# ikergarcia1996/AI-Generated-GTAV

Measured on NVIDIA B200. Metric: generated frames/sec end-to-end (100-step DiT + VAE decode), higher is better.
Workload: dtype bf16

## Files before the change

### ai-generated-gtav_b200/csrc/attn_mma.cu

```cuda
#include <stdlib.h>

#include "attn_seq.cuh"

namespace gtav {

template <int SEQ, int KB, int WARPS, int ROT_PAIRS>
__global__ void __launch_bounds__(WARPS * 32)
attn_seq_kernel(const bf16* __restrict__ qkv, bf16* __restrict__ out, int heads, const float2* __restrict__ rot) {
    __shared__ __align__(16) bf16 sK[KB * SROW];
    __shared__ __align__(16) bf16 sV[KB * SROW];
    pdl_trigger();
    pdl_wait();
    attn_seq_body<SEQ, KB, WARPS, ROT_PAIRS, false>(qkv, out, heads, rot, sK, sV, blockIdx.x, blockIdx.y, blockIdx.z, threadIdx.x, 0);
}

static constexpr int ROT144_BYTES = 144 * 32 * 8;
static constexpr int ATTN144_SMEM = 2 * 144 * SROW * 2 + ROT144_BYTES;
__global__ void __launch_bounds__(3 * 32)
attn_seq144_kernel(const bf16* __restrict__ qkv, bf16* __restrict__ out, int heads, const float2* __restrict__ rot) {
    extern __shared__ __align__(16) uint8_t smem144[];
    bf16* sK = reinterpret_cast<bf16*>(smem144);
    bf16* sV = sK + 144 * SROW;
    float2* sRot = reinterpret_cast<float2*>(smem144 + 2 * 144 * SROW * 2);
    for (int i = threadIdx.x; i < ROT144_BYTES / 16; i += 3 * 32)
        asm volatile("cp.async.cg.shared.global [%0], [%1], 16;" ::"r"(smem_u32(reinterpret_cast<uint8_t*>(sRot) + i * 16)),
                     "l"(reinterpret_cast<const uint8_t*>(rot) + i * 16) : "memory");
    asm volatile("cp.async.commit_group;" ::: "memory");
    pdl_trigger();
    pdl_wait();
    asm volatile("cp.async.wait_group 0;" ::: "memory");
    __syncthreads();
    attn_seq_body<144, 144, 3, 32, false>(qkv, out, heads, sRot, sK, sV, blockIdx.x, blockIdx.y, blockIdx.z, threadIdx.x, 0);
}

static int attn_use_tc(int seq, int groups) {
    const char* e = getenv("GTAV_ATTN");
    if (e != nullptr && e[0] == 't') return 1;
    if (e != nullptr && e[0] == 'm') return 0;
    return seq == 576 ? groups >= 4 : groups >= 96;
}

int launch_attention_seq(const bf16* qkv, bf16* out, int groups, int seq, int heads, const float2* rot, int rot_pairs,
                         cudaStream_t s) {
    if (groups <= 0) return 0;
    if (((seq == 144 && rot_pairs == 32) || (seq == 576 && rot_pairs == 16)) && attn_use_tc(seq, groups))
        return launch_attention_tc(qkv, out, groups, seq, heads, rot, rot_pairs, s);
    if (seq == 144 && rot_pairs == 32) {
        if (groups * heads * 3 <= 2 * 148) {
            static bool configured = false;
            if (!configured) {
                GTAV_CUDA_OK(cudaFuncSetAttribute(attn_seq144_kernel, cudaFuncAttributeMaxDynamicSharedMemorySize, ATTN144_SMEM));
                configured = true;
            }
            GTAV_CUDA_OK(launch_k(attn_seq144_kernel, dim3(3, heads, groups), dim3(3 * 32), ATTN144_SMEM, s, qkv, out, heads, rot));
        } else {
            GTAV_CUDA_OK(launch_k(attn_seq_kernel<144, 144, 3, 32>, dim3(3, heads, groups), dim3(3 * 32), 0, s, qkv, out, heads, rot));
        }
    } else if (seq == 576 && rot_pairs == 16) {
        GTAV_CUDA_OK(launch_k(attn_seq_kernel<576, 64, 4, 16>, dim3(9, heads, groups), dim3(4 * 32), 0, s, qkv, out, heads, rot));
    } else {
        set_error("attention: unsupported (seq=%d, rot_pairs=%d); built for (144,32) and (576,16)", seq, rot_pairs);
        return -1;
    }
    return 0;
}

}
```

### ai-generated-gtav_b200/csrc/attn_seq.cuh

```cuda
#pragma once
#include "common.cuh"
#include "kernels.h"

namespace gtav {

static constexpr int HD = 64;
static constexpr int SROW = HD + 8;

__device__ __forceinline__ void mma_bf16_16816(float (&d)[4], const uint32_t (&a)[4], uint32_t b0, uint32_t b1) {
    asm volatile(
        "mma.sync.aligned.m16n8k16.row.col.f32.bf16.bf16.f32 {%0,%1,%2,%3}, {%4,%5,%6,%7}, {%8,%9}, {%0,%1,%2,%3};"
        : "+f"(d[0]), "+f"(d[1]), "+f"(d[2]), "+f"(d[3])
        : "r"(a[0]), "r"(a[1]), "r"(a[2]), "r"(a[3]), "r"(b0), "r"(b1));
}
__device__ __forceinline__ void ldmatrix_x4_trans(uint32_t (&r)[4], const void* smem_ptr) {
    asm volatile("ldmatrix.sync.aligned.m8n8.x4.trans.shared.b16 {%0,%1,%2,%3}, [%4];"
                 : "=r"(r[0]), "=r"(r[1]), "=r"(r[2]), "=r"(r[3])
                 : "r"(smem_u32(smem_ptr)));
}
__device__ __forceinline__ uint32_t rotate_pair(uint32_t u, float2 cs) {
    const float2 x = unpack_bf16x2(u);
    return pack_bf16x2(x.x * cs.x - x.y * cs.y, x.y * cs.x + x.x * cs.y);
}


__device__ __forceinline__ void attn_bar(int id, int threads) { asm volatile("bar.sync %0, %1;" ::"r"(id), "r"(threads) : "memory"); }
template <bool COHERENT>
__device__ __forceinline__ uint32_t attn_ld32(const bf16* p) {
    if (COHERENT) return __ldcg(reinterpret_cast<const unsigned int*>(p));
    return *reinterpret_cast<const uint32_t*>(p);
}
template <bool COHERENT>
__device__ __forceinline__ uint4 attn_ld128(const bf16* p) {
    if (COHERENT) return __ldcg(reinterpret_cast<const uint4*>(p));
    return *reinterpret_cast<const uint4*>(p);
}

// ... 165 lines not shown
```

### ai-generated-gtav_b200/csrc/dit_engine.cu

```cuda
#include <stdio.h>
#include <stdlib.h>

#include <new>
#include <vector>

#include "../../include/gtav_b200.h"
#include "kernels.h"

using namespace gtav;

struct gtav_dit_s {
    gtav_dit_config cfg;
    gtav_dit_weights w;
    std::vector<gtav_dit_half> halves;
    int tokens;
    int mod_width;
    int patch_k;
    int out_feat;
};

struct Shape {
    int frames = 0, M = 0;
    GemmOp g_patch, g_final;
    std::vector<GemmOp> g_qkv, g_out, g_fc1, g_fc2;
    std::vector<SkinnyOp> s_qkv, s_out, s_fc1, s_fc2;
    bool sk[4] = {false, false, false, false};
    bool fuse_ln = false, fuse_tattn = false;
};

enum BackboneMode { MODE_FULL = 0, MODE_CONTEXT = 1, MODE_LAST = 2 };

struct gtav_dit_plan_s {
    gtav_dit_t eng;
    int B, T, M, R;
    bf16 *xa, *h, *hn, *qkv, *att, *mlp, *yfin, *temb, *aemb, *h1, *cact, *mod;
    bf16* kv_cache;
    float* sk_ws;
    size_t sk_ws_bytes;
    int* sk_counters;
    bool sk_out_of_step = false;
    GemmOp g_t0, g_t2, g_ada;
    Shape full, ctx, last;
// ... 70 lines not shown
    rc |= gemm_prepare(&sh->g_patch, p->xa, 64, static_cast<const bf16*>(w.patch_w), 64, gp(p->h, D, w.patch_b, M, D, 64), EPI_BIAS);
    const int nh = 2 * h->cfg.depth;
    sh->g_qkv.resize(nh); sh->g_out.resize(nh); sh->g_fc1.resize(nh); sh->g_fc2.resize(nh);
    const bool sk_ok = allow_skinny && skinny_enabled() && p->sk_ws != nullptr;
    sh->sk[0] = sk_ok && skinny_pick_splits(M, 3 * D, D) > 0;
    sh->sk[1] = sk_ok && skinny_pick_splits(M, D, D) > 0;
    sh->sk[2] = sk_ok && skinny_pick_splits(M, 4 * D, D) > 0;
    sh->sk[3] = sk_ok && skinny_pick_splits(M, D, 4 * D) > 0;
    if (sh->sk[0]) sh->s_qkv.resize(nh);
    if (sh->sk[1]) sh->s_out.resize(nh);
    if (sh->sk[2]) sh->s_fc1.resize(nh);
    if (sh->sk[3]) sh->s_fc2.resize(nh);
    int so[4] = {0, 0, 0, 0};
    if (const char* e = getenv("GTAV_SK_SPLITS")) sscanf(e, "%d,%d,%d,%d", &so[0], &so[1], &so[2], &so[3]);
    sh->fuse_ln = sh->sk[1] && sh->sk[3] && fuse_enabled();
    sh->fuse_tattn = sh->sk[0] && fuse_enabled() && (so[0] > 0 ? so[0] : skinny_pick_splits(M, 3 * D, D)) == 4 && p->T - 1 <= 7;
    const size_t cache_layer = static_cast<size_t>(p->B) * (p->T - 1) * S * 2 * D;
    for (int i = 0; i < nh && rc == 0; ++i) {
        const gtav_dit_half& hw = h->halves[i];
        const bf16* modl = p->mod + static_cast<size_t>(i) * 6 * D;
        GemmParams pq = gp(p->qkv, 3 * D, nullptr, M, 3 * D, D);
        GemmParams po = gp(p->h, D, hw.out_b, M, D, D);
        po.res = p->h; po.ldr = D; po.gate = modl + 2 * D; po.gate_ld = W; po.rows_per_frame = S;
        GemmParams p1 = gp(p->mlp, 4 * D, hw.fc1_b, M, 4 * D, D);
        GemmParams p2 = gp(p->h, D, hw.fc2_b, M, D, 4 * D);
        p2.res = p->h; p2.ldr = D; p2.gate = modl + 5 * D; p2.gate_ld = W; p2.rows_per_frame = S;
        const size_t DD = static_cast<size_t>(D) * D * 2;
        const char* pfenv = getenv("GTAV_PREFETCH");
        const bool pf_off = pfenv != nullptr && pfenv[0] == '0', pf_force = pfenv != nullptr && pfenv[0] == '1';
        if (!pf_off) {
            if (pf_force || !sh->sk[0]) { pq.prefetch = hw.out_w; pq.prefetch_bytes = DD; }
            if (pf_force || !sh->sk[1]) { po.prefetch = hw.fc1_w; po.prefetch_bytes = 4 * DD; }
            if (pf_force || !sh->sk[2]) { p1.prefetch = hw.fc2_w; p1.prefetch_bytes = 4 * DD; }
            if ((pf_force || !sh->sk[3]) && i + 1 < nh) { p2.prefetch = h->halves[i + 1].qkv_w; p2.prefetch_bytes = 3 * DD; }
        }
        SkinnyFuseParams f_out{}, f_fc2{}, f_qkv{};
        f_out.mode = f_fc2.mode = SK_FUSE_LN;
        f_out.ln_out = f_fc2.ln_out = p->hn;
        f_out.ln_mod = f_fc2.ln_mod = p->mod;
        f_out.ln_mod_ld = f_fc2.ln_mod_ld = W;
        f_out.ln_shift_off = i * 6 * D + 3 * D; f_out.ln_scale_off = i * 6 * D + 4 * D;
        f_fc2.ln_shift_off = (i + 1) * 6 * D; f_fc2.ln_scale_off = (i + 1) * 6 * D + D;
        f_qkv.mode = SK_FUSE_TATTN;
        f_qkv.kv_cache = p->kv_cache + static_cast<size_t>(i >> 1) * cache_layer;
        f_qkv.rot = reinterpret_cast<const float2*>(w.rot_temporal);
        f_qkv.ctx_frames = p->T - 1;
        f_qkv.positions = S;
        const bool ta = sh->fuse_tattn && (i & 1);
        if (ta) { pq.out = p->att; pq.ldo = D; }
        float* ws4[4];
        for (int k = 0; k < 4; ++k) ws4[k] = reinterpret_cast<float*>(reinterpret_cast<uint8_t*>(p->sk_ws) + k * p->sk_ws_bytes);
        const int tag = tag_enabled() ? (2 | ((i & 1) ^ 1)) : 0;
        if (sh->sk[0]) { rc |= skinny_prepare(&sh->s_qkv[i], p->hn, D, static_cast<const bf16*>(hw.qkv_w), D, pq, EPI_STORE, ws4[0], p->sk_counters, so[0], ta ? &f_qkv : nullptr); sh->s_qkv[i].tag = tag; }
        else rc |= gemm_prepare(&sh->g_qkv[i], p->hn, D, static_cast<const bf16*>(hw.qkv_w), D, pq, EPI_STORE);
        if (sh->sk[1]) { rc |= skinny_prepare(&sh->s_out[i], p->att, D, static_cast<const bf16*>(hw.out_w), D, po, EPI_BIAS_GATE_RES, ws4[1], p->sk_counters, so[1], sh->fuse_ln ? &f_out : nullptr); sh->s_out[i].tag = tag; }
        else rc |= gemm_prepare(&sh->g_out[i], p->att, D, static_cast<const bf16*>(hw.out_w), D, po, EPI_BIAS_GATE_RES);
        if (sh->sk[2]) { rc |= skinny_prepare(&sh->s_fc1[i], p->hn, D, static_cast<const bf16*>(hw.fc1_w), D, p1, EPI_BIAS_GELU_TANH, ws4[2], p->sk_counters, so[2]); sh->s_fc1[i].tag = tag; }
        else rc |= gemm_prepare(&sh->g_fc1[i], p->hn, D, static_cast<const bf16*>(hw.fc1_w), D, p1, EPI_BIAS_GELU_TANH);
        if (sh->sk[3]) { rc |= skinny_prepare(&sh->s_fc2[i], p->mlp, 4 * D, static_cast<const bf16*>(hw.fc2_w), 4 * D, p2, EPI_BIAS_GATE_RES, ws4[3], p->sk_counters, so[3], sh->fuse_ln ? &f_fc2 : nullptr); sh->s_fc2[i].tag = tag; }
        else rc |= gemm_prepare(&sh->g_fc2[i], p->mlp, 4 * D, static_cast<const bf16*>(hw.fc2_w), 4 * D, p2, EPI_BIAS_GATE_RES);
    }
    rc |= gemm_prepare(&sh->g_final, p->hn, D, static_cast<const bf16*>(w.final_w), D, gp(p->yfin, 64, w.final_b, M, h->out_feat, D), EPI_BIAS);
    return rc == 0 ? 0 : (rc < 0 ? rc : -1);
}

int run_backbone(gtav_dit_plan_s* p, const Shape* sh, int mode, const void* x, int x_is_bf16, int first_frame,
                 const int* frame_row, void* out, cudaStream_t stream) {
    const gtav_dit_s* e = p->eng;
// ... 13 lines not shown
    if (const char* tr = getenv("GTAV_ENGINE_TRACE")) trace_base = reinterpret_cast<long long*>(strtoull(tr, nullptr, 0));
    int trace_k = 0;
    auto run_skinny = [&](const SkinnyOp& op0) {
        SkinnyOp o = op0;
        o.p.frame_row = frame_row;
        if (trace_base != nullptr) o.trace = trace_base + static_cast<size_t>(trace_k++) * 160 * 8;
        return skinny_run(&o, stream);
    };
    for (int i = 0; i < 2 * c.depth; ++i) {
        const int off = i * 6 * D;
        if (!hn_ready && (rc = launch_ln_modulate(p->h, p->hn, M, D, p->mod, W, off, off + D, frame_row, S, stream))) return rc;
        if (sh->sk[0]) rc = run_skinny(sh->s_qkv[i]);
        else rc = gemm_run(&sh->g_qkv[i], stream);
        if (rc) return rc;
        if (sh->s_qkv.size() && sh->sk[0] && sh->s_qkv[i].f.mode == SK_FUSE_TATTN) {
        } else if ((i & 1) == 0) {
            rc = launch_attention_seq(p->qkv, p->att, F, S, c.heads, rot_s, 32, stream);
        } else {
            bf16* cache = p->kv_cache + static_cast<size_t>(i >> 1) * cache_layer;
            if (mode == MODE_LAST) rc = launch_attention_temporal_last(p->qkv, p->att, p->B, p->T - 1, S, c.heads, rot_t, cache, stream);
            else rc = launch_attention_temporal(p->qkv, p->att, p->B, sh->frames, S, c.heads, rot_t, mode == MODE_CONTEXT ? cache : nullptr, stream);
        }
        if (rc) return rc;
        if (sh->sk[1]) {
            rc = run_skinny(sh->s_out[i]);
        } else {
            GemmOp o = sh->g_out[i];
            o.p.frame_row = frame_row;
            rc = gemm_run(&o, stream);
        }
// ... 208 lines not shown
                                 gtav_stream_t stream) {
    if (!workspace) { set_error("gemm_skinny_tagged: workspace is required"); return -1; }
    if (parity != 0 && parity != 1) { set_error("gemm_skinny_tagged: parity must be 0 or 1, got %d", parity); return -1; }
    return skinny_standalone(A, lda, W, ldw, out, ldo, M, N, K, epilogue, bias, res, ldr, gate, gate_ld, frame_row, rows_per_frame,
                             splits, workspace, nullptr, 2 | parity, stream);
}

int gtav_gemm_skinny_fused_bf16(const void* A, int lda, const void* W, int ldw, void* out, int ldo, int M, int N, int K,
                                const void* bias, const void* res, int ldr, const void* gate, int gate_ld, const int* frame_row,
                                int splits, void* workspace, int* counters, int mode, void* ln_out, const void* ln_mod,
                                int ln_mod_ld, int ln_shift_off, int ln_scale_off, const void* kv_cache, const float* rot,
                                int ctx_frames, int positions, int parity, gtav_stream_t stream) {
    if (!workspace) { set_error("gemm_skinny_fused: workspace is required"); return -1; }
    if (parity < -1 || parity > 1) { set_error("gemm_skinny_fused: parity must be -1, 0 or 1, got %d", parity); return -1; }
    if (parity == -1 && !counters) { set_error("gemm_skinny_fused: counters are required with parity -1"); return -1; }
    if (mode != SK_FUSE_LN && mode != SK_FUSE_TATTN) { set_error("gemm_skinny_fused: mode must be 1 or 2, got %d", mode); return -1; }
    SkinnyFuseParams f{};
    f.mode = mode;
    f.ln_out = static_cast<bf16*>(ln_out);
    f.ln_mod = static_cast<const bf16*>(ln_mod);
    f.ln_mod_ld = ln_mod_ld; f.ln_shift_off = ln_shift_off; f.ln_scale_off = ln_scale_off;
    f.kv_cache = static_cast<const bf16*>(kv_cache);
    f.rot = reinterpret_cast<const float2*>(rot);
    f.ctx_frames = ctx_frames; f.positions = positions;
    const int epi = mode == SK_FUSE_LN ? EPI_BIAS_GATE_RES : EPI_STORE;
    return skinny_standalone(A, lda, W, ldw, out, ldo, M, N, K, epi, bias, res, ldr, gate, gate_ld, frame_row, 144, splits,
                             workspace, parity == -1 ? counters : nullptr, parity == -1 ? 0 : 2 | parity, stream, &f);
}

int gtav_ln_modulate(const void* x, void* out, int M, int D, const void* mod, int mod_ld, int shift_off, int scale_off,
                     const int* frame_row, int rows_per_frame, gtav_stream_t stream) {
    return launch_ln_modulate(static_cast<const bf16*>(x), static_cast<bf16*>(out), M, D, static_cast<const bf16*>(mod),
                              mod_ld, shift_off, scale_off, frame_row, rows_per_frame, stream);
}
int gtav_ln_affine(const void* x, void* out, int M, int D, const float* w, const float* b, gtav_stream_t stream) {
    return launch_ln_affine(static_cast<const bf16*>(x), static_cast<bf16*>(out), M, D, w, b, stream);
}
int gtav_attention_seq(const void* qkv, void* out, int groups, int seq, int heads, const float* rot, int rot_pairs,
                       gtav_stream_t stream) {
    return launch_attention_seq(static_cast<const bf16*>(qkv), static_cast<bf16*>(out), groups, seq, heads,
                                reinterpret_cast<const float2*>(rot), rot_pairs, stream);
}
int gtav_attention_temporal(const void* qkv, void* out, int B, int T, int positions, int heads, const float* rot,
                            gtav_stream_t stream) {
    return launch_attention_temporal(static_cast<const bf16*>(qkv), static_cast<bf16*>(out), B, T, positions, heads,
                                     reinterpret_cast<const float2*>(rot), nullptr, stream);
}
int gtav_attention_temporal_last(const void* qkv, void* out, int B, int ctx_frames, int positions, int heads,
                                 const float* rot, const void* kv_cache, gtav_stream_t stream) {
    return launch_attention_temporal_last(static_cast<const bf16*>(qkv), static_cast<bf16*>(out), B, ctx_frames, positions,
                                          heads, reinterpret_cast<const float2*>(rot), static_cast<const bf16*>(kv_cache), stream);
}
int gtav_ddim_update(const float* x, const void* v_bf16, float* out, int F, int n, const float* abar_t,
                     const float* abar_next, const int* final_flag, gtav_stream_t stream) {
// ... 5 lines not shown
```

### ai-generated-gtav_b200/csrc/gemm_skinny.cu

```cuda
#include "attn_temporal_core.cuh"
#include "common.cuh"
#include "kernels.h"
#include "ln_row.cuh"

namespace gtav {

static constexpr int SK_THREADS = 256;
static constexpr int SK_NT = 144;
static constexpr int SK_W_CHUNK = 128 * 128;
static constexpr int SK_A_CHUNK = SK_NT * 128;
static constexpr int SK_SMEM_BUDGET = 200 * 1024;
static constexpr int SK_TAIL_BYTES = 128 + 4096 + 2048;
static constexpr int SK_TMAX = 7;

struct SkinnyParams {
    GemmParams g;
    SkinnyFuseParams f;
    int splits, chunks, tiles;
    int gemm_ctas;
    float* ws;
    int* counters;
    int tag;
    long long* trace;
};
// ... 126 lines not shown
        y[3] = r1.y + bf16_round(g1.y * y[3]);
    }
    uint2 o;
    o.x = pack_bf16x2(y[0], y[1]);
    o.y = pack_bf16x2(y[2], y[3]);
    return o;
}
template <int EPI>
__device__ __noinline__ void skinny_store4(const GemmParams& g, int tok, int n, float4 acc, uint2 bias) {
    Epi4Ops e;
    if (EPI == EPI_BIAS_GATE_RES) e = skinny_epi4_load<EPI>(g, tok, n);
    e.bias = bias;
    *reinterpret_cast<uint2*>(g.out + static_cast<size_t>(tok) * g.ldo + n) = skinny_epi4<EPI>(acc, e);
}

template <int EPI, int S>
__device__ __forceinline__ void skinny_reduce(const GemmParams& g, const float* part, int total, int lo, int hi, int wid, int lane,
                                              int n0, uint2 bias, SkTag tg) {
    static_assert(S <= 4, "the unrolled reduce is instantiated for S = 4 only; other split counts use skinny_reduce_any");
    const float* base = part + 4 * lane;
    const uint32_t keep = ~tg.chk;
    constexpr int IT = 5;
#pragma unroll 1
    for (int t0 = lo + wid; t0 < hi; t0 += 8 * IT) {
        uint4 v[IT][S];
        uint32_t pending = 0u, spins = 0u;
#pragma unroll
        for (int it = 0; it < IT; ++it)
#pragma unroll
            for (int s2 = 0; s2 < S; ++s2)
                if (t0 + 8 * it < hi) v[it][s2] = ld_relaxed_u4(base + (static_cast<size_t>(s2) * total + t0 + 8 * it) * 128);
#pragma unroll
        for (int it = 0; it < IT; ++it)
#pragma unroll
            for (int s2 = 0; s2 < S; ++s2)
                if (t0 + 8 * it < hi && !tag_ok(v[it][s2], tg)) pending |= 1u << (S * it + s2);
        while (pending) {
            tag_spin_check(spins);
#pragma unroll
            for (int it = 0; it < IT; ++it)
#pragma unroll
// ... 4 lines not shown
#pragma unroll
                for (int s2 = 0; s2 < S; ++s2)
                    if ((pending >> (S * it + s2) & 1u) && tag_ok(v[it][s2], tg)) pending &= ~(1u << (S * it + s2));
        }
#pragma unroll
        for (int it = 0; it < IT; ++it) {
            const int tok = t0 + 8 * it;
            if (tok < hi) {
                float4 acc = make_float4(__uint_as_float(v[it][0].x & keep), __uint_as_float(v[it][0].y & keep),
                                         __uint_as_float(v[it][0].z & keep), __uint_as_float(v[it][0].w & keep));
#pragma unroll
                for (int s2 = 1; s2 < S; ++s2) {
                    acc.x += __uint_as_float(v[it][s2].x & keep); acc.y += __uint_as_float(v[it][s2].y & keep);
                    acc.z += __uint_as_float(v[it][s2].z & keep); acc.w += __uint_as_float(v[it][s2].w & keep);
                }
                skinny_store4<EPI>(g, tok, n0 + 4 * lane, acc, bias);
            }
        }
    }
}

template <int S>
__device__ __forceinline__ float4 skinny_sum4(const float* p0, size_t stride, SkTag tg) {
    uint4 v[S];
    const uint32_t keep = ~tg.chk;
    uint32_t pending = 0u, spins = 0u;
#pragma unroll
    for (int s2 = 0; s2 < S; ++s2) v[s2] = ld_relaxed_u4(p0 + s2 * stride);
#pragma unroll
    for (int s2 = 0; s2 < S; ++s2)
        if (!tag_ok(v[s2], tg)) pending |= 1u << s2;
// ... 171 lines not shown
    extern __shared__ uint8_t smem_raw[];
    uint8_t* smem = reinterpret_cast<uint8_t*>((reinterpret_cast<uintptr_t>(smem_raw) + 1023) & ~uintptr_t(1023));
    const int chunks = p.chunks, tiles = p.tiles, S = p.splits;
    uint8_t* sW = smem;
    uint8_t* sA = smem + chunks * SK_W_CHUNK;
    uint8_t* tail = sA + tiles * chunks * SK_A_CHUNK;
    uint64_t* bar_w = reinterpret_cast<uint64_t*>(tail);
    uint64_t* bar_a = bar_w + 1;
    uint64_t* bar_acc = bar_w + 6;
    uint32_t* tmem_slot = reinterpret_cast<uint32_t*>(bar_w + 7);
    uint8_t* smod = tail + 128;
    uint8_t* srow = smod + 4096;

    const int warp = threadIdx.x >> 5, lane = threadIdx.x & 31;
    if (threadIdx.x == 128) SK_STAMP(0);
    const bool gemm_cta = FUSE == SK_FUSE_NONE || static_cast<int>(blockIdx.x) < p.gemm_ctas;
    const int rb = blockIdx.x / S, split = blockIdx.x - rb * S;
    const int kc0 = split * chunks;
    const int total = tiles * SK_NT;
    const uint32_t tmem_cols = total <= 256 ? 256u : 512u;
    const bool tagged = p.tag != 0;
    SkTag tg;
    tg.chk = tagged ? 1u : 0u;
    tg.par = tagged ? static_cast<uint32_t>(p.tag & 1) : 0u;

    if (gemm_cta && warp == 0 && lane == 0) {
        tma_prefetch_desc(&tmW);
        mbar_init(bar_w, 1);
        mbar_init(bar_acc, 1);
        fence_barrier_init();
        mbar_arrive_expect_tx(bar_w, chunks * SK_W_CHUNK);
// ... 42 lines not shown
#pragma unroll
                    for (int k = 0; k < 4; ++k)
                        umma_bf16_ss(tmem_base + t * SK_NT, dw + 2 * k, da + 2 * k, idesc, (ch | k) != 0 ? 1u : 0u);
                }
                __syncwarp();
                dw += SK_W_CHUNK >> 4;
                da += SK_A_CHUNK >> 4;
            }
        }
        if (elect_one()) umma_commit(bar_acc);
        __syncwarp();
        pdl_wait();
    } else {
        pdl_wait();
    }
    int* const meet = tagged ? nullptr : p.counters + 4 * (FUSE == SK_FUSE_NONE ? rb : 64);
    const int meet_n = FUSE == SK_FUSE_NONE ? S : static_cast<int>(gridDim.x);
    int sense0 = 0;
    if (threadIdx.x == 128 && meet_n > 1 && !tagged) sense0 = ld_acquire_gpu(meet + 2);
    Epi4Ops epre;
    epre.bias = epre.gate = epre.res = make_uint2(0u, 0u);
    TattnPre tpre;
    if (FUSE == SK_FUSE_LN) {
        if (static_cast<int>(blockIdx.x) < total) epre = skinny_ln_preload(p, blockIdx.x, warp, smod);
    } else if (FUSE == SK_FUSE_TATTN) {
        if (static_cast<int>(blockIdx.x) < total) skinny_tattn_preload(p, blockIdx.x, warp, lane, tpre);
    } else if (EPI != EPI_STORE && S > 1) {
        epre.bias = *reinterpret_cast<const uint2*>(p.g.bias + rb * 128 + 4 * lane);
    }

    if (FUSE == SK_FUSE_NONE && S == 1 && warp >= 4) {
        const GemmParams& g = p.g;
        const int q = warp & 3;
        const int n = rb * 128 + q * 32 + lane;
        float bias_n = 0.f;
        if (EPI != EPI_STORE) bias_n = __bfloat162float(g.bias[n]);
        mbar_wait(bar_acc, 0);
        tcgen05_fence_after();
        const uint32_t tlane = tmem_base + (static_cast<uint32_t>(q * 32) << 16);
#pragma unroll 1
        for (int c = 0; c < total; c += 16) {
            uint32_t v[16];
            tmem_ld_32x16(tlane + c, v);
            tmem_ld_wait();
#pragma unroll
            for (int i = 0; i < 16; ++i) skinny_store<EPI>(g, c + i, n, __uint_as_float(v[i]), bias_n);
// ... 42 lines not shown
            if (threadIdx.x == 128) SK_STAMP(5);
            const long long t0 = clock64();
            tcgen05_fence_before();
            if (warp == 2) {
                asm volatile("bar.sync 1, 256;" ::: "memory");
                tcgen05_fence_after();
                tmem_dealloc(tmem_base, tmem_cols);
            } else {
                asm volatile("bar.arrive 1, 256;" ::: "memory");
            }
            if (GTAV_SK_TAG_DELAY > 0) {
                while (clock64() - t0 < GTAV_SK_TAG_DELAY) {}
            }
            if (threadIdx.x == 128) SK_STAMP(6);
        }
    } else if (FUSE != SK_FUSE_NONE && !tagged && threadIdx.x == 128) {
        skinny_rendezvous(meet, meet_n, sense0);
    } else if (FUSE != SK_FUSE_NONE && tagged) {
        if (threadIdx.x == 0 && static_cast<int>(blockIdx.x) < total) {
            const float* probe = p.ws + (static_cast<size_t>(p.gemm_ctas - 1) * total + blockIdx.x) * 128 + 127;
            uint32_t spins = 0u;
            while (!tag_ok(ld_relaxed_u1(probe), tg)) tag_spin_check(spins);
        }
        __syncthreads();
    }
    if (S > 1 && FUSE == SK_FUSE_NONE) {
        if (!tagged) {
            __syncthreads();
            if (threadIdx.x == 128) SK_STAMP(6);
        }
        const GemmParams& g = p.g;
        const int lo = split * total / S, hi = (split + 1) * total / S;
        const float* part = p.ws + static_cast<size_t>(rb) * S * total * 128;
        if (S == 4) skinny_reduce<EPI, 4>(g, part, total, lo, hi, warp, lane, rb * 128, epre.bias, tg);
        else skinny_reduce_any<EPI>(g, part, S, total, lo, hi, warp, lane, rb * 128, epre.bias, tg);
        if (threadIdx.x == 128) SK_STAMP(7);
    }
    if (FUSE != SK_FUSE_NONE) {
        if (!tagged) {
            __syncthreads();
            if (threadIdx.x == 128) SK_STAMP(6);
        }
        if (FUSE == SK_FUSE_LN) {
            skinny_reduce_ln(p, S, total, warp, lane, smod, srow, epre, tg);
        } else {
            skinny_reduce_tattn<4>(p, total, warp, lane, tpre, tg);
        }
        if (threadIdx.x == 128) SK_STAMP(7);
    }
    if (S == 1 && gemm_cta) {
        tcgen05_fence_before();
        __syncthreads();
        if (warp == 2) tmem_dealloc(tmem_base, tmem_cols);
// ... 52 lines not shown
    op->splits = S;
    op->chunks = kchunks / S;
    op->tiles = tiles;
    op->ws = ws;
    op->counters = counters;
    op->trace = nullptr;
    op->tag = 0;
    op->f = SkinnyFuseParams{};
    op->grid = rbs * S;
    if (fuse != nullptr && fuse->mode != SK_FUSE_NONE) {
        const bool ln_ok = fuse->mode == SK_FUSE_LN && epi == EPI_BIAS_GATE_RES && p.N == 1024 && (S == 4 || S == 8 || S == 16) && fuse->ln_out != nullptr &&
                           fuse->ln_mod != nullptr && fuse->ln_mod_ld % 8 == 0 && fuse->ln_shift_off % 8 == 0 && fuse->ln_scale_off % 8 == 0;
        const bool ta_ok = fuse->mode == SK_FUSE_TATTN && epi == EPI_STORE && p.N == 3072 && S == 4 && fuse->rot != nullptr &&
                           fuse->ctx_frames >= 0 && fuse->ctx_frames <= 7 && (fuse->ctx_frames == 0 || fuse->kv_cache != nullptr) &&
                           fuse->positions > 0 && p.M % fuse->positions == 0;
        if (!ln_ok && !ta_ok) {
            set_error("skinny gemm: fused reduce mode %d does not fit M=%d N=%d K=%d epi=%d splits=%d", fuse->mode, p.M, p.N, p.K, epi, S);
            return -1;
        }
        op->f = *fuse;
        int sms = 148, dev = 0, n = 0;
        if (cudaGetDevice(&dev) == cudaSuccess && cudaDeviceGetAttribute(&n, cudaDevAttrMultiProcessorCount, dev) == cudaSuccess && n > 0) sms = n;
        const int want = p.M < sms ? p.M : sms;
        if (want > op->grid) op->grid = want;
    }
    int rc = make_tmap_3d(&op->tmW, W, p.N, p.K, ldw, 128, op->chunks);
    if (rc) return rc;
    return make_tmap_3d(&op->tmA, A, p.M, p.K, lda, SK_NT, op->chunks);
}

template <int EPI, int FUSE>
static int skinny_launch(const SkinnyOp* op, cudaStream_t stream) {
    static bool configured = false;
    auto kern = gemm_skinny_kernel<EPI, FUSE>;
    if (!configured) {
// ... 2 lines not shown
    }
    SkinnyParams sp;
    sp.g = op->p; sp.f = op->f; sp.splits = op->splits; sp.chunks = op->chunks; sp.tiles = op->tiles; sp.ws = op->ws;
    sp.counters = op->counters; sp.gemm_ctas = (op->p.N / 128) * op->splits;
    sp.trace = op->trace;
    sp.tag = op->tag;
    size_t smem = static_cast<size_t>(op->chunks) * (SK_W_CHUNK + op->tiles * SK_A_CHUNK) + SK_TAIL_BYTES + 1024;
    if (smem < 120 * 1024) smem = 120 * 1024;
    GTAV_CUDA_OK(launch_k(kern, dim3(op->grid), dim3(SK_THREADS), smem, stream, op->tmW, op->tmA, sp));
    return 0;
}

int skinny_run(const SkinnyOp* op, cudaStream_t stream) {
    if (op->f.mode == SK_FUSE_LN) return skinny_launch<EPI_BIAS_GATE_RES, SK_FUSE_LN>(op, stream);
    if (op->f.mode == SK_FUSE_TATTN) return skinny_launch<EPI_STORE, SK_FUSE_TATTN>(op, stream);
    switch (op->epi) {
        case EPI_STORE: return skinny_launch<EPI_STORE, SK_FUSE_NONE>(op, stream);
        case EPI_BIAS: return skinny_launch<EPI_BIAS, SK_FUSE_NONE>(op, stream);
        case EPI_BIAS_GELU_TANH: return skinny_launch<EPI_BIAS_GELU_TANH, SK_FUSE_NONE>(op, stream);
        case EPI_BIAS_GATE_RES: return skinny_launch<EPI_BIAS_GATE_RES, SK_FUSE_NONE>(op, stream);
    }
    set_error("skinny gemm: unknown epilogue %d", op->epi);
    return -1;
}

}
```

### ai-generated-gtav_b200/csrc/kernels.h

```cpp
#pragma once
#include <cuda.h>
#include <cuda_bf16.h>
#include <cuda_runtime.h>
#include <stdint.h>

namespace gtav {

typedef __nv_bfloat16 bf16;

void set_error(const char* fmt, ...);
const char* get_error();
#define GTAV_CUDA_OK(expr)                                                                     \
    do {                                                                                       \
        cudaError_t e__ = (expr);                                                              \
        if (e__ != cudaSuccess) {                                                              \
            gtav::set_error("%s failed: %s (%s:%d)", #expr, cudaGetErrorString(e__), __FILE__, __LINE__); \
            return -2;                                                                         \
        }                                                                                      \
    } while (0)

bool pdl_enabled();
template <typename... KArgs, typename... Args>
inline cudaError_t launch_k(void (*kern)(KArgs...), dim3 grid, dim3 block, size_t smem, cudaStream_t stream, Args&&... args) {
    cudaLaunchConfig_t cfg{};
// ... 43 lines not shown
    int kc;
    int epi;
};

int gemm_prepare(GemmOp* op, const bf16* A, int lda, const bf16* W, int ldw, const GemmParams& p, int epi,
                 int bn_override = 0);
int gemm_run(const GemmOp* op, cudaStream_t stream);
bool gemm2_eligible(int M, int N, int K);
int gemm2_run(const GemmOp* op, cudaStream_t stream);
bool gemm_splitk_eligible(int M, int N, int K, int sms);
int gemm_splitk_run(const GemmOp* op, cudaStream_t stream);

int make_tmap_3d(CUtensorMap* out, const bf16* ptr, uint64_t rows, uint64_t cols, uint64_t ld, uint32_t box_rows,
                 uint32_t box_chunks);

enum SkinnyFuse : int { SK_FUSE_NONE = 0, SK_FUSE_LN = 1, SK_FUSE_TATTN = 2 };
struct SkinnyFuseParams {
    int mode;
    bf16* ln_out;
    const bf16* ln_mod;
    int ln_mod_ld, ln_shift_off, ln_scale_off;
    const bf16* kv_cache;
    const float2* rot;
    int ctx_frames, positions;
};
struct SkinnyOp {
    CUtensorMap tmW, tmA;
    GemmParams p;
    SkinnyFuseParams f;
    int grid;
    int epi, splits, chunks, tiles;
// ... 3 lines not shown
    long long* trace;
};
bool skinny_supported(int M, int N, int K, int epi);
int skinny_pick_splits(int M, int N, int K);
size_t skinny_workspace_bytes(int M);
int skinny_prepare(SkinnyOp* op, const bf16* A, int lda, const bf16* W, int ldw, const GemmParams& p, int epi, float* ws,
                   int* counters, int splits_override = 0, const SkinnyFuseParams* fuse = nullptr);
int skinny_run(const SkinnyOp* op, cudaStream_t stream);

int launch_ln_modulate(const bf16* x, bf16* out, int M, int D, const bf16* mod, int mod_ld, int shift_off,
                       int scale_off, const int* frame_row, int rows_per_frame, cudaStream_t s);
int launch_ln_affine(const bf16* x, bf16* out, int M, int D, const float* w, const float* b, cudaStream_t s);

int launch_attention_seq(const bf16* qkv, bf16* out, int groups, int seq, int heads, const float2* rot, int rot_pairs,
                         cudaStream_t s);
int launch_attention_tc(const bf16* qkv, bf16* out, int groups, int seq, int heads, const float2* rot, int rot_pairs,
                        cudaStream_t s);
int launch_attention_temporal(const bf16* qkv, bf16* out, int B, int T, int positions, int heads, const float2* rot,
                              bf16* kv_cache, cudaStream_t s);
int launch_attention_temporal_last(const bf16* qkv, bf16* out, int B, int ctx_frames, int positions, int heads,
                                   const float2* rot, const bf16* kv_cache, cudaStream_t s);

int launch_cond_prep(const int64_t* t, const float* actions, int act_dim, int R, const float* freqs, const bf16* Wa,
                     const bf16* ba, bf16* temb, bf16* aemb, int D, cudaStream_t s);
int launch_patchify(const void* x, int x_is_bf16, bf16* out, int ldo, int F, int C, int H, int W, int p,
                    int frames_per_group, long group_stride, cudaStream_t s);
int launch_dit_unpatchify(const bf16* y, bf16* out, int F, int C, int gh, int gw, int p, cudaStream_t s);
int launch_vae_unpatchify(const bf16* y, void* out, int to_u8, int F, int sh, int sw, int p, cudaStream_t s);
int launch_cast_pad(const float* z, bf16* out, int rows, int C, int ldo, float scale, cudaStream_t s);
int launch_take_mean(const bf16* moments, int ldm, float* out, int rows, int C, float scale, int round_bf16,
// ... 10 lines not shown
```

Baseline: 10.03.

## Fuse spatial RoPE into skinny QKV reduce and add key-split seq-144 attention

Adds a new seq-144 spatial attention kernel that splits the keys across three warps, each handling 48 keys, and merges the partial softmax results through shared memory, with a finer grid (9 query blocks per head). Adds a skinny-GEMM fusion mode that applies the spatial rotary rotation to the Q/K columns during the split-K reduce, so the attention kernel can skip the rotation. The engine turns both on whenever the QKV skinny GEMM uses 4 splits. This is meant to cut attention latency and rotation work per step, at the cost of an extra cross-warp merge and rounding the rotated values to bf16 at a different point.

```diff
diff --git a/ai-generated-gtav_b200/csrc/attn_mma.cu b/ai-generated-gtav_b200/csrc/attn_mma.cu
--- a/ai-generated-gtav_b200/csrc/attn_mma.cu
+++ b/ai-generated-gtav_b200/csrc/attn_mma.cu
@@ -33,6 +33,176 @@
     attn_seq_body<144, 144, 3, 32, false>(qkv, out, heads, sRot, sK, sV, blockIdx.x, blockIdx.y, blockIdx.z, threadIdx.x, 0);
 }
 
+static constexpr int A144_KEYS = 48;
+template <bool ROTATE>
+__global__ void __launch_bounds__(3 * 32)
+attn_seq144_split_kernel(const bf16* __restrict__ qkv, bf16* __restrict__ out, int heads, const float2* __restrict__ rot) {
+    __shared__ __align__(16) bf16 sK[144 * SROW];
+    __shared__ __align__(16) bf16 sV[144 * SROW];
+    __shared__ __align__(16) bf16 sQ[3][16 * SROW];
+    const int warp = threadIdx.x >> 5, lane = threadIdx.x & 31;
+    const int g = lane >> 2, tig = lane & 3;
+    const int q0 = blockIdx.x * 16, head = blockIdx.y, k0 = warp * A144_KEYS;
+    const int ld = 3 * heads * HD;
+    const bf16* qbase = qkv + static_cast<size_t>(blockIdx.z) * 144 * ld + head * HD;
+    const bf16* kbase = qbase + heads * HD;
+    const bf16* vbase = kbase + heads * HD;
+    bf16* myQ = sQ[warp];
+    bf16* myK = sK + k0 * SROW;
+    bf16* myV = sV + k0 * SROW;
+    constexpr int QC = 16 * 8 / 32, KC = A144_KEYS * 8 / 32;
+    float4 cs[QC + KC][2];
+    if (ROTATE) {
+#pragma unroll
+        for (int i = 0; i < QC + KC; ++i) {
+            const int idx = lane + 32 * (i < QC ? i : i - QC);
+            const int r = (i < QC ? q0 : k0) + (idx >> 3), c8 = (idx & 7) * 8;
+            const float4* t = reinterpret_cast<const float4*>(rot + r * 32 + (c8 >> 1));
+            cs[i][0] = __ldg(t);
+            cs[i][1] = __ldg(t + 1);
+        }
+    }
+    pdl_trigger();
+    pdl_wait();
+#pragma unroll
+    for (int i = 0; i < QC + KC; ++i) {
+        const int idx = lane + 32 * (i < QC ? i : i - QC);
+        const int r = idx >> 3, c8 = (idx & 7) * 8;
+        const bf16* src = i < QC ? qbase + static_cast<size_t>(q0 + r) * ld + c8 : kbase + static_cast<size_t>(k0 + r) * ld + c8;
+        bf16* dst = (i < QC ? myQ : myK) + r * SROW + c8;
+        asm volatile("cp.async.cg.shared.global [%0], [%1], 16;" ::"r"(smem_u32(dst)), "l"(src) : "memory");
+    }
+    asm volatile("cp.async.commit_group;" ::: "memory");
+#pragma unroll
+    for (int i = 0; i < KC; ++i) {
+        const int idx = lane + 32 * i;
+        const int r = idx >> 3, c8 = (idx & 7) * 8;
+        asm volatile("cp.async.cg.shared.global [%0], [%1], 16;" ::"r"(smem_u32(myV + r * SROW + c8)),
+                     "l"(vbase + static_cast<size_t>(k0 + r) * ld + c8) : "memory");
+    }
+    asm volatile("cp.async.commit_group;" ::: "memory");
+    asm volatile("cp.async.wait_group 1;" ::: "memory");
+    if (ROTATE) {
+#pragma unroll
+        for (int i = 0; i < QC + KC; ++i) {
+            const int idx = lane + 32 * (i < QC ? i : i - QC);
+            const int r = idx >> 3, c8 = (idx & 7) * 8;
+            uint4* p = reinterpret_cast<uint4*>((i < QC ? myQ : myK) + r * SROW + c8);
+            uint4 x = *p;
+            x.x = rotate_pair(x.x, make_float2(cs[i][0].x, cs[i][0].y));
+            x.y = rotate_pair(x.y, make_float2(cs[i][0].z, cs[i][0].w));
+            x.z = rotate_pair(x.z, make_float2(cs[i][1].x, cs[i][1].y));
+            x.w = rotate_pair(x.w, make_float2(cs[i][1].z, cs[i][1].w));
+            *p = x;
+        }
+    }
+    __syncwarp();
+
+    uint32_t qf[4][4];
+#pragma unroll
+    for (int ks = 0; ks < 4; ++ks)
+#pragma unroll
+        for (int h = 0; h < 4; ++h)
+            qf[ks][h] = *reinterpret_cast<const uint32_t*>(myQ + (g + (h & 1) * 8) * SROW + ks * 16 + 2 * tig + (h >> 1) * 8);
+    float sc[A144_KEYS / 8][4];
+#pragma unroll
+    for (int nt = 0; nt < A144_KEYS / 8; ++nt) {
+#pragma unroll
+        for (int j = 0; j < 4; ++j) sc[nt][j] = 0.f;
+#pragma unroll
+        for (int ks = 0; ks < 4; ++ks) {
+            const bf16* kp = myK + (nt * 8 + g) * SROW + ks * 16 + 2 * tig;
+            mma_bf16_16816(sc[nt], qf[ks], *reinterpret_cast<const uint32_t*>(kp), *reinterpret_cast<const uint32_t*>(kp + 8));
+        }
+    }
+    const float sl2 = 0.125f * 1.4426950408889634f;
+    float m[2] = {-INFINITY, -INFINITY}, l[2] = {0.f, 0.f};
+#pragma unroll
+    for (int nt = 0; nt < A144_KEYS / 8; ++nt) {
+        m[0] = fmaxf(m[0], fmaxf(sc[nt][0], sc[nt][1]));
+        m[1] = fmaxf(m[1], fmaxf(sc[nt][2], sc[nt][3]));
+    }
+#pragma unroll
+    for (int h = 0; h < 2; ++h) {
+        m[h] = fmaxf(m[h], __shfl_xor_sync(0xffffffffu, m[h], 1));
+        m[h] = fmaxf(m[h], __shfl_xor_sync(0xffffffffu, m[h], 2));
+    }
+    const float mo0 = m[0] * sl2, mo1 = m[1] * sl2;
+#pragma unroll
+    for (int nt = 0; nt < A144_KEYS / 8; ++nt) {
+        sc[nt][0] = exp2f(sc[nt][0] * sl2 - mo0);
+        sc[nt][1] = exp2f(sc[nt][1] * sl2 - mo0);
+        sc[nt][2] = exp2f(sc[nt][2] * sl2 - mo1);
+        sc[nt][3] = exp2f(sc[nt][3] * sl2 - mo1);
+        l[0] += sc[nt][0] + sc[nt][1];
+        l[1] += sc[nt][2] + sc[nt][3];
+    }
+#pragma unroll
+    for (int h = 0; h < 2; ++h) {
+        l[h] += __shfl_xor_sync(0xffffffffu, l[h], 1);
+        l[h] += __shfl_xor_sync(0xffffffffu, l[h], 2);
+    }
+    float o[8][4];
+#pragma unroll
+    for (int i = 0; i < 8; ++i)
+#pragma unroll
+        for (int j = 0; j < 4; ++j) o[i][j] = 0.f;
+    asm volatile("cp.async.wait_group 0;" ::: "memory");
+    __syncwarp();
+#pragma unroll
+    for (int j = 0; j < A144_KEYS / 16; ++j) {
+        uint32_t pf[4];
+        pf[0] = pack_bf16x2(sc[2 * j][0], sc[2 * j][1]);
+        pf[1] = pack_bf16x2(sc[2 * j][2], sc[2 * j][3]);
+        pf[2] = pack_bf16x2(sc[2 * j + 1][0], sc[2 * j + 1][1]);
+        pf[3] = pack_bf16x2(sc[2 * j + 1][2], sc[2 * j + 1][3]);
+#pragma unroll
+        for (int dn = 0; dn < 8; dn += 2) {
+            const int mat = lane >> 3, r = lane & 7;
+            uint32_t vf[4];
+            ldmatrix_x4_trans(vf, myV + (j * 16 + (mat & 1) * 8 + r) * SROW + (dn + (mat >> 1)) * 8);
+            mma_bf16_16816(o[dn], pf, vf[0], vf[1]);
+            mma_bf16_16816(o[dn + 1], pf, vf[2], vf[3]);
+        }
+    }
+    if (warp > 0) {
+        float4* x = reinterpret_cast<float4*>(myK);
+#pragma unroll
+        for (int i = 0; i < 8; ++i) x[i * 32 + lane] = make_float4(o[i][0], o[i][1], o[i][2], o[i][3]);
+        x[8 * 32 + lane] = make_float4(m[0], m[1], l[0], l[1]);
+    }
+    __syncthreads();
+    if (warp > 0) return;
+    const float4* x1 = reinterpret_cast<const float4*>(sK + A144_KEYS * SROW);
+    const float4* x2 = reinterpret_cast<const float4*>(sK + 2 * A144_KEYS * SROW);
+    const float4 ml1 = x1[8 * 32 + lane], ml2 = x2[8 * 32 + lane];
+    float a[3][2], inv[2];
+    {
+        const float mm[3][2] = {{m[0], m[1]}, {ml1.x, ml1.y}, {ml2.x, ml2.y}};
+        const float ll[3][2] = {{l[0], l[1]}, {ml1.z, ml1.w}, {ml2.z, ml2.w}};
+#pragma unroll
+        for (int h = 0; h < 2; ++h) {
+            const float mx = fmaxf(fmaxf(mm[0][h], mm[1][h]), mm[2][h]);
+#pragma unroll
+            for (int w = 0; w < 3; ++w) a[w][h] = exp2f((mm[w][h] - mx) * sl2);
+            inv[h] = 1.0f / (ll[0][h] * a[0][h] + ll[1][h] * a[1][h] + ll[2][h] * a[2][h]);
+        }
+    }
+    const int ldo = heads * HD;
+    bf16* obase = out + (static_cast<size_t>(blockIdx.z) * 144 + q0) * ldo + head * HD;
+#pragma unroll
+    for (int dn = 0; dn < 8; ++dn) {
+        const float4 y1 = x1[dn * 32 + lane], y2 = x2[dn * 32 + lane];
+        const float r0 = o[dn][0] * a[0][0] + y1.x * a[1][0] + y2.x * a[2][0];
+        const float r1 = o[dn][1] * a[0][0] + y1.y * a[1][0] + y2.y * a[2][0];
+        const float r2 = o[dn][2] * a[0][1] + y1.z * a[1][1] + y2.z * a[2][1];
+        const float r3 = o[dn][3] * a[0][1] + y1.w * a[1][1] + y2.w * a[2][1];
+        const int c = dn * 8 + 2 * tig;
+        *reinterpret_cast<uint32_t*>(obase + static_cast<size_t>(g) * ldo + c) = pack_bf16x2(r0 * inv[0], r1 * inv[0]);
+        *reinterpret_cast<uint32_t*>(obase + static_cast<size_t>(g + 8) * ldo + c) = pack_bf16x2(r2 * inv[1], r3 * inv[1]);
+    }
+}
+
 static int attn_use_tc(int seq, int groups) {
     const char* e = getenv("GTAV_ATTN");
     if (e != nullptr && e[0] == 't') return 1;
@@ -43,6 +213,8 @@
 int launch_attention_seq(const bf16* qkv, bf16* out, int groups, int seq, int heads, const float2* rot, int rot_pairs,
                          cudaStream_t s) {
     if (groups <= 0) return 0;
+    const char* e = getenv("GTAV_ATTN");
+    if (seq == 144 && rot_pairs == 32 && e != nullptr && e[0] == 's') return launch_attention_seq144_split(qkv, out, groups, heads, rot, s);
     if (((seq == 144 && rot_pairs == 32) || (seq == 576 && rot_pairs == 16)) && attn_use_tc(seq, groups))
         return launch_attention_tc(qkv, out, groups, seq, heads, rot, rot_pairs, s);
     if (seq == 144 && rot_pairs == 32) {
@@ -65,4 +237,11 @@
     return 0;
 }
 
-}
+int launch_attention_seq144_split(const bf16* qkv, bf16* out, int groups, int heads, const float2* rot, cudaStream_t s) {
+    if (groups <= 0) return 0;
+    if (rot != nullptr) GTAV_CUDA_OK(launch_k(attn_seq144_split_kernel<true>, dim3(9, heads, groups), dim3(3 * 32), 0, s, qkv, out, heads, rot));
+    else GTAV_CUDA_OK(launch_k(attn_seq144_split_kernel<false>, dim3(9, heads, groups), dim3(3 * 32), 0, s, qkv, out, heads, rot));
+    return 0;
+}
+
+}
diff --git a/ai-generated-gtav_b200/csrc/attn_seq.cuh b/ai-generated-gtav_b200/csrc/attn_seq.cuh
--- a/ai-generated-gtav_b200/csrc/attn_seq.cuh
+++ b/ai-generated-gtav_b200/csrc/attn_seq.cuh
@@ -20,7 +20,7 @@
 }
 __device__ __forceinline__ uint32_t rotate_pair(uint32_t u, float2 cs) {
     const float2 x = unpack_bf16x2(u);
-    return pack_bf16x2(x.x * cs.x - x.y * cs.y, x.y * cs.x + x.x * cs.y);
+    return pack_bf16x2(__fmaf_rn(x.x, cs.x, -__fmul_rn(x.y, cs.y)), __fmaf_rn(x.y, cs.x, __fmul_rn(x.x, cs.y)));
 }
 
 
diff --git a/ai-generated-gtav_b200/csrc/dit_engine.cu b/ai-generated-gtav_b200/csrc/dit_engine.cu
--- a/ai-generated-gtav_b200/csrc/dit_engine.cu
+++ b/ai-generated-gtav_b200/csrc/dit_engine.cu
@@ -25,7 +25,8 @@
     std::vector<GemmOp> g_qkv, g_out, g_fc1, g_fc2;
     std::vector<SkinnyOp> s_qkv, s_out, s_fc1, s_fc2;
     bool sk[4] = {false, false, false, false};
-    bool fuse_ln = false, fuse_tattn = false;
+    bool fuse_ln = false, fuse_tattn = false, fuse_rot = false;
+    bool attn_split = false;
 };
 
 enum BackboneMode { MODE_FULL = 0, MODE_CONTEXT = 1, MODE_LAST = 2 };
@@ -126,7 +127,9 @@
     int so[4] = {0, 0, 0, 0};
     if (const char* e = getenv("GTAV_SK_SPLITS")) sscanf(e, "%d,%d,%d,%d", &so[0], &so[1], &so[2], &so[3]);
     sh->fuse_ln = sh->sk[1] && sh->sk[3] && fuse_enabled();
-    sh->fuse_tattn = sh->sk[0] && fuse_enabled() && (so[0] > 0 ? so[0] : skinny_pick_splits(M, 3 * D, D)) == 4 && p->T - 1 <= 7;
+    sh->attn_split = sh->sk[0] && (so[0] > 0 ? so[0] : skinny_pick_splits(M, 3 * D, D)) == 4;
+    sh->fuse_rot = sh->attn_split && fuse_enabled();
+    sh->fuse_tattn = sh->fuse_rot && p->T - 1 <= 7;
     const size_t cache_layer = static_cast<size_t>(p->B) * (p->T - 1) * S * 2 * D;
     for (int i = 0; i < nh && rc == 0; ++i) {
         const gtav_dit_half& hw = h->halves[i];
@@ -146,7 +149,7 @@
             if (pf_force || !sh->sk[2]) { p1.prefetch = hw.fc2_w; p1.prefetch_bytes = 4 * DD; }
             if ((pf_force || !sh->sk[3]) && i + 1 < nh) { p2.prefetch = h->halves[i + 1].qkv_w; p2.prefetch_bytes = 3 * DD; }
         }
-        SkinnyFuseParams f_out{}, f_fc2{}, f_qkv{};
+        SkinnyFuseParams f_out{}, f_fc2{}, f_qkv{}, f_rot{};
         f_out.mode = f_fc2.mode = SK_FUSE_LN;
         f_out.ln_out = f_fc2.ln_out = p->hn;
         f_out.ln_mod = f_fc2.ln_mod = p->mod;
@@ -158,12 +161,15 @@
         f_qkv.rot = reinterpret_cast<const float2*>(w.rot_temporal);
         f_qkv.ctx_frames = p->T - 1;
         f_qkv.positions = S;
+        f_rot.mode = SK_FUSE_ROT;
+        f_rot.rot = reinterpret_cast<const float2*>(w.rot_spatial);
         const bool ta = sh->fuse_tattn && (i & 1);
+        const SkinnyFuseParams* fq = ta ? &f_qkv : (sh->fuse_rot && !(i & 1) ? &f_rot : nullptr);
         if (ta) { pq.out = p->att; pq.ldo = D; }
         float* ws4[4];
         for (int k = 0; k < 4; ++k) ws4[k] = reinterpret_cast<float*>(reinterpret_cast<uint8_t*>(p->sk_ws) + k * p->sk_ws_bytes);
         const int tag = tag_enabled() ? (2 | ((i & 1) ^ 1)) : 0;
-        if (sh->sk[0]) { rc |= skinny_prepare(&sh->s_qkv[i], p->hn, D, static_cast<const bf16*>(hw.qkv_w), D, pq, EPI_STORE, ws4[0], p->sk_counters, so[0], ta ? &f_qkv : nullptr); sh->s_qkv[i].tag = tag; }
+        if (sh->sk[0]) { rc |= skinny_prepare(&sh->s_qkv[i], p->hn, D, static_cast<const bf16*>(hw.qkv_w), D, pq, EPI_STORE, ws4[0], p->sk_counters, so[0], fq); sh->s_qkv[i].tag = tag; }
         else rc |= gemm_prepare(&sh->g_qkv[i], p->hn, D, static_cast<const bf16*>(hw.qkv_w), D, pq, EPI_STORE);
         if (sh->sk[1]) { rc |= skinny_prepare(&sh->s_out[i], p->att, D, static_cast<const bf16*>(hw.out_w), D, po, EPI_BIAS_GATE_RES, ws4[1], p->sk_counters, so[1], sh->fuse_ln ? &f_out : nullptr); sh->s_out[i].tag = tag; }
         else rc |= gemm_prepare(&sh->g_out[i], p->att, D, static_cast<const bf16*>(hw.out_w), D, po, EPI_BIAS_GATE_RES);
@@ -207,6 +213,8 @@
         else rc = gemm_run(&sh->g_qkv[i], stream);
         if (rc) return rc;
         if (sh->s_qkv.size() && sh->sk[0] && sh->s_qkv[i].f.mode == SK_FUSE_TATTN) {
+        } else if ((i & 1) == 0 && sh->attn_split) {
+            rc = launch_attention_seq144_split(p->qkv, p->att, F, c.heads, sh->s_qkv[i].f.mode == SK_FUSE_ROT ? nullptr : rot_s, stream);
         } else if ((i & 1) == 0) {
             rc = launch_attention_seq(p->qkv, p->att, F, S, c.heads, rot_s, 32, stream);
         } else {
@@ -445,7 +453,10 @@
     if (!workspace) { set_error("gemm_skinny_fused: workspace is required"); return -1; }
     if (parity < -1 || parity > 1) { set_error("gemm_skinny_fused: parity must be -1, 0 or 1, got %d", parity); return -1; }
     if (parity == -1 && !counters) { set_error("gemm_skinny_fused: counters are required with parity -1"); return -1; }
-    if (mode != SK_FUSE_LN && mode != SK_FUSE_TATTN) { set_error("gemm_skinny_fused: mode must be 1 or 2, got %d", mode); return -1; }
+    if (mode != SK_FUSE_LN && mode != SK_FUSE_TATTN && mode != SK_FUSE_ROT) {
+        set_error("gemm_skinny_fused: mode must be 1, 2 or 3, got %d", mode);
+        return -1;
+    }
     SkinnyFuseParams f{};
     f.mode = mode;
     f.ln_out = static_cast<bf16*>(ln_out);
@@ -469,6 +480,10 @@
 }
 int gtav_attention_seq(const void* qkv, void* out, int groups, int seq, int heads, const float* rot, int rot_pairs,
                        gtav_stream_t stream) {
+    if (rot == nullptr) {
+        if (seq != 144) { set_error("attention_seq: q / k arrive rotated (rot NULL) for seq 144 only, got %d", seq); return -1; }
+        return launch_attention_seq144_split(static_cast<const bf16*>(qkv), static_cast<bf16*>(out), groups, heads, nullptr, stream);
+    }
     return launch_attention_seq(static_cast<const bf16*>(qkv), static_cast<bf16*>(out), groups, seq, heads,
                                 reinterpret_cast<const float2*>(rot), rot_pairs, stream);
 }
diff --git a/ai-generated-gtav_b200/csrc/gemm_skinny.cu b/ai-generated-gtav_b200/csrc/gemm_skinny.cu
--- a/ai-generated-gtav_b200/csrc/gemm_skinny.cu
+++ b/ai-generated-gtav_b200/csrc/gemm_skinny.cu
@@ -1,3 +1,4 @@
+#include "attn_seq.cuh"
 #include "attn_temporal_core.cuh"
 #include "common.cuh"
 #include "kernels.h"
@@ -164,9 +165,19 @@
     *reinterpret_cast<uint2*>(g.out + static_cast<size_t>(tok) * g.ldo + n) = skinny_epi4<EPI>(acc, e);
 }
 
-template <int EPI, int S>
+__device__ __forceinline__ void skinny_store4_rot(const GemmParams& g, int tok, int n, float4 acc, bool rotq, float4 cs) {
+    Epi4Ops e;
+    uint2 o = skinny_epi4<EPI_STORE>(acc, e);
+    if (rotq) {
+        o.x = rotate_pair(o.x, make_float2(cs.x, cs.y));
+        o.y = rotate_pair(o.y, make_float2(cs.z, cs.w));
+    }
+    *reinterpret_cast<uint2*>(g.out + static_cast<size_t>(tok) * g.ldo + n) = o;
+}
+
+template <int EPI, int S, bool ROT = false>
 __device__ __forceinline__ void skinny_reduce(const GemmParams& g, const float* part, int total, int lo, int hi, int wid, int lane,
-                                              int n0, uint2 bias, SkTag tg) {
+                                              int n0, uint2 bias, SkTag tg, const float2* rot = nullptr) {
     static_assert(S <= 4, "the unrolled reduce is instantiated for S = 4 only; other split counts use skinny_reduce_any");
     const float* base = part + 4 * lane;
     const uint32_t keep = ~tg.chk;
@@ -175,6 +186,13 @@
     for (int t0 = lo + wid; t0 < hi; t0 += 8 * IT) {
         uint4 v[IT][S];
         uint32_t pending = 0u, spins = 0u;
+        const bool rotq = ROT && n0 < 2048;
+        float4 cs[IT];
+        if (rotq) {
+#pragma unroll
+            for (int it = 0; it < IT; ++it)
+                if (t0 + 8 * it < hi) cs[it] = __ldg(reinterpret_cast<const float4*>(rot + ((t0 + 8 * it) % SK_NT) * 32 + (((n0 + 4 * lane) & 63) >> 1)));
+        }
 #pragma unroll
         for (int it = 0; it < IT; ++it)
 #pragma unroll
@@ -209,7 +227,8 @@
                     acc.x += __uint_as_float(v[it][s2].x & keep); acc.y += __uint_as_float(v[it][s2].y & keep);
                     acc.z += __uint_as_float(v[it][s2].z & keep); acc.w += __uint_as_float(v[it][s2].w & keep);
                 }
-                skinny_store4<EPI>(g, tok, n0 + 4 * lane, acc, bias);
+                if (ROT) skinny_store4_rot(g, tok, n0 + 4 * lane, acc, rotq, cs[it]);
+                else skinny_store4<EPI>(g, tok, n0 + 4 * lane, acc, bias);
             }
         }
     }
@@ -411,7 +430,8 @@
 
     const int warp = threadIdx.x >> 5, lane = threadIdx.x & 31;
     if (threadIdx.x == 128) SK_STAMP(0);
-    const bool gemm_cta = FUSE == SK_FUSE_NONE || static_cast<int>(blockIdx.x) < p.gemm_ctas;
+    constexpr bool ROWS = FUSE == SK_FUSE_LN || FUSE == SK_FUSE_TATTN;
+    const bool gemm_cta = !ROWS || static_cast<int>(blockIdx.x) < p.gemm_ctas;
     const int rb = blockIdx.x / S, split = blockIdx.x - rb * S;
     const int kc0 = split * chunks;
     const int total = tiles * SK_NT;
@@ -484,8 +504,8 @@
     } else {
         pdl_wait();
     }
-    int* const meet = tagged ? nullptr : p.counters + 4 * (FUSE == SK_FUSE_NONE ? rb : 64);
-    const int meet_n = FUSE == SK_FUSE_NONE ? S : static_cast<int>(gridDim.x);
+    int* const meet = tagged ? nullptr : p.counters + 4 * (!ROWS ? rb : 64);
+    const int meet_n = !ROWS ? S : static_cast<int>(gridDim.x);
     int sense0 = 0;
     if (threadIdx.x == 128 && meet_n > 1 && !tagged) sense0 = ld_acquire_gpu(meet + 2);
     Epi4Ops epre;
@@ -499,7 +519,7 @@
         epre.bias = *reinterpret_cast<const uint2*>(p.g.bias + rb * 128 + 4 * lane);
     }
 
-    if (FUSE == SK_FUSE_NONE && S == 1 && warp >= 4) {
+    if (!ROWS && S == 1 && warp >= 4) {
         const GemmParams& g = p.g;
         const int q = warp & 3;
         const int n = rb * 128 + q * 32 + lane;
@@ -572,9 +592,9 @@
             }
             if (threadIdx.x == 128) SK_STAMP(6);
         }
-    } else if (FUSE != SK_FUSE_NONE && !tagged && threadIdx.x == 128) {
+    } else if (ROWS && !tagged && threadIdx.x == 128) {
         skinny_rendezvous(meet, meet_n, sense0);
-    } else if (FUSE != SK_FUSE_NONE && tagged) {
+    } else if (ROWS && tagged) {
         if (threadIdx.x == 0 && static_cast<int>(blockIdx.x) < total) {
             const float* probe = p.ws + (static_cast<size_t>(p.gemm_ctas - 1) * total + blockIdx.x) * 128 + 127;
             uint32_t spins = 0u;
@@ -582,7 +602,7 @@
         }
         __syncthreads();
     }
-    if (S > 1 && FUSE == SK_FUSE_NONE) {
+    if (S > 1 && !ROWS) {
         if (!tagged) {
             __syncthreads();
             if (threadIdx.x == 128) SK_STAMP(6);
@@ -590,11 +610,12 @@
         const GemmParams& g = p.g;
         const int lo = split * total / S, hi = (split + 1) * total / S;
         const float* part = p.ws + static_cast<size_t>(rb) * S * total * 128;
-        if (S == 4) skinny_reduce<EPI, 4>(g, part, total, lo, hi, warp, lane, rb * 128, epre.bias, tg);
+        if (FUSE == SK_FUSE_ROT) skinny_reduce<EPI, 4, true>(g, part, total, lo, hi, warp, lane, rb * 128, epre.bias, tg, p.f.rot);
+        else if (S == 4) skinny_reduce<EPI, 4>(g, part, total, lo, hi, warp, lane, rb * 128, epre.bias, tg);
         else skinny_reduce_any<EPI>(g, part, S, total, lo, hi, warp, lane, rb * 128, epre.bias, tg);
         if (threadIdx.x == 128) SK_STAMP(7);
     }
-    if (FUSE != SK_FUSE_NONE) {
+    if (ROWS) {
         if (!tagged) {
             __syncthreads();
             if (threadIdx.x == 128) SK_STAMP(6);
@@ -677,11 +698,14 @@
         const bool ta_ok = fuse->mode == SK_FUSE_TATTN && epi == EPI_STORE && p.N == 3072 && S == 4 && fuse->rot != nullptr &&
                            fuse->ctx_frames >= 0 && fuse->ctx_frames <= 7 && (fuse->ctx_frames == 0 || fuse->kv_cache != nullptr) &&
                            fuse->positions > 0 && p.M % fuse->positions == 0;
-        if (!ln_ok && !ta_ok) {
+        const bool rot_ok = fuse->mode == SK_FUSE_ROT && epi == EPI_STORE && p.N == 3072 && S == 4 && fuse->rot != nullptr;
+        if (!ln_ok && !ta_ok && !rot_ok) {
             set_error("skinny gemm: fused reduce mode %d does not fit M=%d N=%d K=%d epi=%d splits=%d", fuse->mode, p.M, p.N, p.K, epi, S);
             return -1;
         }
         op->f = *fuse;
+    }
+    if (fuse != nullptr && (fuse->mode == SK_FUSE_LN || fuse->mode == SK_FUSE_TATTN)) {
         int sms = 148, dev = 0, n = 0;
         if (cudaGetDevice(&dev) == cudaSuccess && cudaDeviceGetAttribute(&n, cudaDevAttrMultiProcessorCount, dev) == cudaSuccess && n > 0) sms = n;
         const int want = p.M < sms ? p.M : sms;
@@ -714,6 +738,7 @@
 int skinny_run(const SkinnyOp* op, cudaStream_t stream) {
     if (op->f.mode == SK_FUSE_LN) return skinny_launch<EPI_BIAS_GATE_RES, SK_FUSE_LN>(op, stream);
     if (op->f.mode == SK_FUSE_TATTN) return skinny_launch<EPI_STORE, SK_FUSE_TATTN>(op, stream);
+    if (op->f.mode == SK_FUSE_ROT) return skinny_launch<EPI_STORE, SK_FUSE_ROT>(op, stream);
     switch (op->epi) {
         case EPI_STORE: return skinny_launch<EPI_STORE, SK_FUSE_NONE>(op, stream);
         case EPI_BIAS: return skinny_launch<EPI_BIAS, SK_FUSE_NONE>(op, stream);
diff --git a/ai-generated-gtav_b200/csrc/kernels.h b/ai-generated-gtav_b200/csrc/kernels.h
--- a/ai-generated-gtav_b200/csrc/kernels.h
+++ b/ai-generated-gtav_b200/csrc/kernels.h
@@ -81,7 +81,7 @@
 int make_tmap_3d(CUtensorMap* out, const bf16* ptr, uint64_t rows, uint64_t cols, uint64_t ld, uint32_t box_rows,
                  uint32_t box_chunks);
 
-enum SkinnyFuse : int { SK_FUSE_NONE = 0, SK_FUSE_LN = 1, SK_FUSE_TATTN = 2 };
+enum SkinnyFuse : int { SK_FUSE_NONE = 0, SK_FUSE_LN = 1, SK_FUSE_TATTN = 2, SK_FUSE_ROT = 3 };
 struct SkinnyFuseParams {
     int mode;
     bf16* ln_out;
@@ -115,6 +115,7 @@
 
 int launch_attention_seq(const bf16* qkv, bf16* out, int groups, int seq, int heads, const float2* rot, int rot_pairs,
                          cudaStream_t s);
+int launch_attention_seq144_split(const bf16* qkv, bf16* out, int groups, int heads, const float2* rot, cudaStream_t s);
 int launch_attention_tc(const bf16* qkv, bf16* out, int groups, int seq, int heads, const float2* rot, int rot_pairs,
                         cudaStream_t s);
 int launch_attention_temporal(const bf16* qkv, bf16* out, int B, int T, int positions, int heads, const float2* rot,
```

New measurement: 10.16, median of 6. 1.3% higher.
